# stormalex/minimap2_chaindp

Hardware: AMD Instinct MI355X
Metric: chained anchors/sec (whole node) (higher is better)
Workload: dtype int32

## Files before the change

minimap2_chaindp_amd/csrc/chaindp_lanes.h:

```cpp
#ifndef CHAINDP_LANES_H
#define CHAINDP_LANES_H

#include <hip/hip_runtime.h>
#include <stdint.h>

namespace chaindp {

#if defined(__HIP_DEVICE_COMPILE__)
#define TW_LDS(T, a) ((__attribute__((address_space(3))) T*)(a))
#else
#define TW_LDS(T, a) ((T*)(uintptr_t)(a))
#endif
#if defined(__HIP_DEVICE_COMPILE__)
#define TW_CONST(T, p) ((const __attribute__((address_space(4))) T*)(uintptr_t)(p))
#else
#define TW_CONST(T, p) ((const T*)(p))
#endif
typedef uint32_t tw_u32x2 __attribute__((ext_vector_type(2)));
typedef uint32_t tw_u32x4 __attribute__((ext_vector_type(4)));

__device__ __forceinline__ tw_u32x2 tw_ld64(uint32_t a) { return *TW_LDS(const tw_u32x2, a); }
__device__ __forceinline__ int tw_ld32(uint32_t a) { return *TW_LDS(const int, a); }
__device__ __forceinline__ int tw_ld_i8(uint32_t a) { return (int)*TW_LDS(const signed char, a); }
__device__ __forceinline__ int tw_ld_u8(uint32_t a) { return (int)*TW_LDS(const unsigned char, a); }
__device__ __forceinline__ tw_u32x4 tw_ld128(uint32_t a) { return *TW_LDS(const tw_u32x4, a); }
__device__ __forceinline__ void tw_st64(uint32_t a, uint32_t x, uint32_t y) { tw_u32x2 t; t.x = x; t.y = y; *TW_LDS(tw_u32x2, a) = t; }
__device__ __forceinline__ void tw_st32(uint32_t a, int v) { *TW_LDS(int, a) = v; }
__device__ __forceinline__ void tw_st8(uint32_t a, int v) { *TW_LDS(signed char, a) = (signed char)v; }
__device__ __forceinline__ void tw_st128(uint32_t a, uint32_t x, uint32_t y, uint32_t z, uint32_t w) { tw_u32x4 t; t.x = x; t.y = y; t.z = z; t.w = w; *TW_LDS(tw_u32x4, a) = t; }

#if defined(__HIP_DEVICE_COMPILE__)
#define TW_VREG(x) asm volatile("" : "+v"(x))
#else
#define TW_VREG(x) ((void)(x))
#endif

#define TW_UNI(x) ((uint32_t)__builtin_amdgcn_readfirstlane((int)(x)))

__device__ __forceinline__ uint32_t tw_sad(uint32_t a, uint32_t b, uint32_t c)
{
	uint32_t d = 0;
#if defined(__HIP_DEVICE_COMPILE__)
	asm("v_sad_u32 %0, %1, %2, %3" : "=v"(d) : "v"(a), "v"(b), "v"(c));
#endif
	return d;
}

__device__ __forceinline__ uint32_t tw_absdiff(uint32_t a, uint32_t b)
{
	uint32_t d = 0;
#if defined(__HIP_DEVICE_COMPILE__)
	asm("v_sad_u32 %0, %1, %2, 0" : "=v"(d) : "v"(a), "v"(b));
#endif
	return d;
}

__device__ __forceinline__ uint32_t tw_sub_m1(uint32_t b, uint32_t a)
{
	uint32_t d = 0;
#if defined(__HIP_DEVICE_COMPILE__)
	asm("v_xad_u32 %0, %1, -1, %2" : "=v"(d) : "v"(a), "v"(b));
#endif
	return d;
}

#define TW_ULT(a, b) __builtin_amdgcn_uicmp((unsigned)(a), (unsigned)(b), 36)
#define TW_EQ(a, b)  __builtin_amdgcn_uicmp((unsigned)(a), (unsigned)(b), 32)
#define TW_SGT(a, b) __builtin_amdgcn_sicmp((int)(a), (int)(b), 38)
#define TW_SGE(a, b) __builtin_amdgcn_sicmp((int)(a), (int)(b), 39)
#define TW_SEL(m, a, b) (__builtin_amdgcn_inverse_ballot_w64(m) ? (a) : (b))

}
#endif
```

minimap2_chaindp_amd/csrc/chaindp_twin.hip:

```cpp
#include <hip/hip_runtime.h>
#include <stdint.h>
#include <limits.h>
#include <stdio.h>
#include <stdlib.h>
#include <vector>
#include "chaindp_kernels.h"
#include "chaindp_wave.h"
#include "chaindp_lanes.h"

namespace chaindp {

#define TW_XY 0u
#define TW_PF 2048u
#define TW_V 3072u
#define TW_LUT_BYTES 512u
#define TW_ST_HALF 56u
#define TW_MK_HALF 260u
template <bool ONE_LUT> struct TwLayout {
	static constexpr bool HAS_XQ = !ONE_LUT;
	static constexpr uint32_t XQ = 3584u, XQ_HALF = 512u;
	static constexpr uint32_t LUT = ONE_LUT ? 3584u : XQ + 2u * XQ_HALF;
	static constexpr uint32_t LUT_HALF = ONE_LUT ? 0u : TW_LUT_BYTES;
	static constexpr uint32_t ST = LUT + (ONE_LUT ? 1u : 2u) * TW_LUT_BYTES;
	static constexpr uint32_t MK = ST + 2u * TW_ST_HALF;
	static constexpr uint32_t SP = MK + 2u * TW_MK_HALF;
	static constexpr uint32_t SP_HALF = ONE_LUT ? 0u : 64u;
	static constexpr uint32_t SP_OF_XQ = SP - XQ / 8u;
	static constexpr uint32_t KEY = SP + 128u;
	static constexpr uint32_t KEY_HALF = ONE_LUT ? 0u : 4u;
	static constexpr uint32_t BYTES = KEY + 8u;
	static_assert(ST % 8u == 0u && MK % 4u == 0u && KEY % 4u == 0u, "cold state is read as 64-bit words, marks and keys as 32-bit");
};
static_assert(TwLayout<true>::BYTES == 4864u && TwLayout<true>::BYTES <= 5120u, "one table: 32 workgroups per CU");
static_assert(TwLayout<false>::BYTES == 6400u, "two tables: 24 workgroups per CU");
template <bool SAMEGAP, bool ONE_LUT> struct TwWaves { static constexpr int N = !ONE_LUT ? 6 : SAMEGAP ? 8 : 7; };
#define TW_TILE 64
#define TW_RING 64
#define TW_QCH 8

__device__ __forceinline__ int tw_excl_max32(int v)
{
	v = max(v, __builtin_amdgcn_update_dpp(0, v, DPP_ROW_SHR(1), 0xf, 0xf, true));
	v = max(v, __builtin_amdgcn_update_dpp(0, v, DPP_ROW_SHR(2), 0xf, 0xf, true));
	v = max(v, __builtin_amdgcn_update_dpp(0, v, DPP_ROW_SHR(4), 0xf, 0xf, true));
	v = max(v, __builtin_amdgcn_update_dpp(0, v, DPP_ROW_SHR(8), 0xf, 0xf, true));
	int e = __builtin_amdgcn_update_dpp(0, v, DPP_ROW_SHR(1), 0xf, 0xf, true);
#if defined(__HIP_DEVICE_COMPILE__)
	asm("s_nop 1\n\tv_max_i32_dpp %0, %1, %0 row_bcast:15 row_mask:0xa bank_mask:0xf" : "+v"(e) : "v"(v));
#endif
	return e;
}
__device__ __forceinline__ int tw_incl_min32(int v)
{
	v = min(v, dpp_or_old<DPP_ROW_SHR(1), 0xf>(INT_MAX, v));
	v = min(v, dpp_or_old<DPP_ROW_SHR(2), 0xf>(INT_MAX, v));
	v = min(v, dpp_or_old<DPP_ROW_SHR(4), 0xf>(INT_MAX, v));
	v = min(v, dpp_or_old<DPP_ROW_SHR(8), 0xf>(INT_MAX, v));
	v = min(v, dpp_or_old<DPP_ROW_BCAST15, 0xa>(INT_MAX, v));
	return v;
}

__device__ __forceinline__ int tw_below_in_half(uint64_t m, bool hi_half)
{
	const int lo = (int)__builtin_amdgcn_mbcnt_lo((uint32_t)m, 0u);
	const int hi = (int)__builtin_amdgcn_mbcnt_hi((uint32_t)(m >> 32), 0u);
	return hi_half ? hi : lo;
}

__device__ __forceinline__ uint64_t tw_smear_halves(uint64_t m)
{
	uint32_t lo = 0, hi = 0;
#if defined(__HIP_DEVICE_COMPILE__)
	asm("s_cmp_lg_u32 %2, 0\n\ts_cselect_b32 %0, -1, 0\n\ts_cmp_lg_u32 %3, 0\n\ts_cselect_b32 %1, -1, 0"
	    : "=&s"(lo), "=&s"(hi) : "s"(TW_UNI((uint32_t)m)), "s"(TW_UNI((uint32_t)(m >> 32))) : "scc");
#endif
	return (uint64_t)hi << 32 | lo;
}

__device__ __forceinline__ uint64_t tw_last_or_lane0(uint64_t m)
{
	uint32_t lo = 0, hi = 0;
#if defined(__HIP_DEVICE_COMPILE__)
	asm("s_flbit_i32_b32 %0, %2\n\ts_flbit_i32_b32 %1, %3\n\ts_lshr_b32 %0, 0x80000000, %0\n\ts_lshr_b32 %1, 0x80000000, %1"
	    : "=&s"(lo), "=&s"(hi) : "s"(TW_UNI((uint32_t)m)), "s"(TW_UNI((uint32_t)(m >> 32))));
#endif
	return (uint64_t)hi << 32 | lo;
}

__device__ __forceinline__ uint32_t tw_both_halves(uint64_t m)
{
	uint32_t t = 0;
#if defined(__HIP_DEVICE_COMPILE__)
	asm("s_cmp_lg_u32 %1, 0\n\ts_cselect_b32 %0, %2, 0" : "=s"(t) : "s"(TW_UNI((uint32_t)m)), "s"(TW_UNI((uint32_t)(m >> 32))) : "scc");
#endif
	return t;
}

__device__ __forceinline__ uint64_t tw_below_first(uint64_t m, uint64_t b)
{
	const uint32_t blo = (uint32_t)b, bhi = (uint32_t)(b >> 32);
	const uint32_t klo = blo ? (blo & (0u - blo)) - 1u : 0xffffffffu, khi = bhi ? (bhi & (0u - bhi)) - 1u : 0xffffffffu;
	return m & ((uint64_t)khi << 32 | klo);
}

#define TW_HI31 0x8000000080000000ull

struct TwinArgs {
	Params par;
	const int64_t *off;
	const ulonglong2 *a;
	const unsigned long long *sumq;
	const uint16_t *lut;
	int lut_stride;
	const Unit *units;
	const UnitAux *aux;
	const unsigned long long *counters;
	int32_t *f, *p, *v;
	int32_t *first_child;
	uint8_t *flags;
	Unit *left;
	unsigned int *left_cnt;
	unsigned int *queue;
	const unsigned int *key_range;
	unsigned int *route;
	int two_tables;
	int force_left;
	int64_t total;
	unsigned long long *stamp;
};

struct TwinCold {
	int64_t next;
	int64_t base;
	uint64_t x_carry;
	int32_t rel0, room, read, tile0;
};

struct TwinHot {
	uint32_t S;
	uint32_t m4;
	uint32_t pc;
	uint32_t pend;
};
#define TW_CARRY 40u

#ifdef CHAINDP_TWIN_STAMPS
#define TW_STAMP(...) __VA_ARGS__
#else
#define TW_STAMP(...)
#endif
#if defined(CHAINDP_TWIN_STAMPS) && CHAINDP_TWIN_STAMPS == 2
#define TW_STAMP_A(...)
#define TW_STAMP_B(...) __VA_ARGS__
#elif defined(CHAINDP_TWIN_STAMPS) && CHAINDP_TWIN_STAMPS == 1
#define TW_STAMP_A(...) __VA_ARGS__
#define TW_STAMP_B(...)
#else
#define TW_STAMP_A(...)
#define TW_STAMP_B(...)
#endif
#if defined(CHAINDP_TWIN_STAMPS) && CHAINDP_TWIN_STAMPS == 3
#define TW_STAMP_C(...) __VA_ARGS__
#else
#define TW_STAMP_C(...)
#endif
#define TW_NOW() __builtin_amdgcn_s_memtime()

template <bool SAMEGAP, bool ONE_LUT>
__global__ __launch_bounds__(64) __attribute__((amdgpu_waves_per_eu(TwWaves<SAMEGAP, ONE_LUT>::N, TwWaves<SAMEGAP, ONE_LUT>::N))) void k_chain_twin(TwinArgs g)
{
	using L = TwLayout<ONE_LUT>;
	const int lane = threadIdx.x;
	const bool hi_half = lane >= 32;
	const int h = lane >> 5, hl = lane & 31;

	uint32_t L16 = (uint32_t)hl << 4;
	const uint32_t mkbase = L::MK + TW_MK_HALF * (uint32_t)h;
	const uint32_t curbase = L::XQ + L::XQ_HALF * (uint32_t)h;
	uint32_t c_mkbase = mkbase;
	uint32_t c_far = mkbase + 256u;
	uint32_t c_own = mkbase + ((uint32_t)hl << 2);
	uint32_t c_lut = ONE_LUT ? 0u : L::LUT + L::LUT_HALF * (uint32_t)h;
	uint32_t c_8h = (uint32_t)h << 3;
	uint32_t c_M = (uint32_t)g.par.max_dist_x;
	uint32_t c_bw = (uint32_t)g.par.bw;
	uint32_t c_cbw = c_M - 1u > c_bw ? c_M - 1u - c_bw : 0u;
	const uint32_t mdq = (uint32_t)(g.par.max_dist_x < g.par.max_dist_y ? g.par.max_dist_x : g.par.max_dist_y);
	uint32_t c_dqoff = c_M - mdq;
	int c_ms = g.par.max_skip;
	int c_min = INT_MIN;
	int c_Mout = hl == 31 ? g.par.max_dist_x : INT_MAX;
	uint32_t c_bwl = c_bw + c_lut;
	uint32_t c_cbwl = c_cbw - c_lut;
	constexpr uint32_t LUT_OFF = ONE_LUT ? L::LUT : 0u;
	TW_VREG(L16); TW_VREG(c_far); TW_VREG(c_own);
	if (!ONE_LUT) { TW_VREG(c_M); TW_VREG(c_ms); }
	if (!ONE_LUT) TW_VREG(c_lut);
	if (!SAMEGAP) TW_VREG(c_dqoff);
	TW_VREG(c_min); TW_VREG(c_Mout); TW_VREG(c_bwl); TW_VREG(c_cbwl);

	const uint64_t maxx = (uint64_t)(int64_t)g.par.max_dist_x;
	const uint32_t route = *g.route;
	if (ONE_LUT ? route == 1u || g.key_range[0] != g.key_range[1] || g.two_tables : route == 1u || route == 2u) return;
	const int64_t n_units = (int64_t)(uint32_t)g.counters[0];
	const int64_t n_single = (int64_t)(g.counters[0] >> 32);
	const bool short_units = (g.total - n_single) <= 512 * n_units;
	if (!short_units) {
		if (blockIdx.x == 0 && lane == 0) *g.left_cnt = 0xffffffffu;
		return;
	}
	if (blockIdx.x == 0 && lane == 0) *g.route = ONE_LUT ? 2u : 3u;
	const bool params_ok = g.lut != nullptr && !g.par.is_cdna && g.par.max_dist_x >= 1 && g.par.max_dist_y >= 0 &&
	                       ((uint64_t)(int64_t)g.par.max_dist_x + 1) * 129ull < (1ull << 31) && g.par.bw + 1 <= (int)TW_LUT_BYTES && g.force_left != 1;

	TwinHot u;
	u.S = 0; u.m4 = 0; u.pc = L::HAS_XQ ? curbase : 0u; u.pend = u.pc;
	uint64_t live_m = ~0ull;
	uint64_t contm = 0;
	const uint32_t st_addr = L::ST + TW_ST_HALF * (uint32_t)h;
#define TW_COLD (*TW_LDS(TwinCold, st_addr))
	const uint32_t xcd = blockIdx.x & 7u;
	const uint32_t n_halves = 2u * gridDim.x;
#ifndef TW_END_UNITS
#define TW_END_UNITS 16u
#define TW_PIECE 1u
#endif
	const uint32_t U1 = n_units > (long long)TW_END_UNITS * n_halves ? ((uint32_t)n_units - TW_END_UNITS * n_halves) & ~(8u * TW_QCH - 1u) : 0u;
	const uint32_t G1k = U1 / (8u * TW_QCH);
	auto grab = [&](uint32_t p, uint32_t &nx, uint32_t &ne) {
		if (p < G1k) { nx = (8u * p + xcd) * TW_QCH; ne = nx + TW_QCH; }
		else { nx = U1 + TW_PIECE * (8u * (p - G1k) + xcd); ne = nx + TW_PIECE; }
	};
	if (hl == 0) {
		uint32_t nx, ne;
		grab(((blockIdx.x >> 3) << 1) | (uint32_t)h, nx, ne);
		tw_st64(st_addr, nx, ne); tw_st64(st_addr + 8u, 0u, 0u);
		tw_st64(st_addr + 16u, 0u, 0u); tw_st64(st_addr + 24u, 0u, 0u);
		tw_st64(st_addr + 32u, 0u, (uint32_t)-TW_TILE);
		tw_st64(st_addr + TW_CARRY, 0xfffffffcu, 0u); tw_st64(st_addr + TW_CARRY + 8u, 0u, 0u);
		tw_st32(L::KEY + 4u * (uint32_t)h, -1);
	}
	wave_mem_fence();

	constexpr bool PF = !ONE_LUT;
	uint64_t nx0_x = 0, nx0_y = 0, nx1_x = 0, nx1_y = 0;
	int32_t pfu0 = -1, pfu1 = -1;

	TW_STAMP(unsigned long long st_t0 = 0; unsigned int st_service = 0, st_n_service = 0, st_n_fast = 0, st_flush = 0, st_unit = 0, st_n_unit = 0, st_head = 0, st_take = 0, st_tail = 0;)

	auto service = [&](uint64_t svc) {
#if defined(__HIP_DEVICE_COMPILE__)
		asm volatile("s_waitcnt vmcnt(0)" ::: "memory");
#endif
		wave_mem_fence();
		uint64_t retired = 0;
		for (int hs = 0; hs < 2; ++hs) {
			if (((svc >> (32 * hs)) & 1ull) == 0) continue;
			TW_STAMP_B(const unsigned long long th0 = g.stamp ? TW_NOW() : 0;)
			const uint64_t hm = hs ? 0xffffffff00000000ull : 0x00000000ffffffffull;
			const uint32_t sa = L::ST + TW_ST_HALF * (uint32_t)hs, keya = L::KEY + L::KEY_HALF * (uint32_t)hs;
			const uint32_t mkb = L::MK + TW_MK_HALF * (uint32_t)hs, lutb = L::LUT + L::LUT_HALF * (uint32_t)hs;
			const uint32_t curb = L::XQ + L::XQ_HALF * (uint32_t)hs, spb = L::SP + L::SP_HALF * (uint32_t)hs;
			const tw_u32x2 cw0 = tw_ld64(sa), cw1 = tw_ld64(sa + 8u), cw2 = tw_ld64(sa + 16u), cw3 = tw_ld64(sa + 24u), cw4 = tw_ld64(sa + 32u);
			int64_t c_next = (int64_t)((uint64_t)TW_UNI(cw0.y) << 32 | TW_UNI(cw0.x));
			int64_t c_base = (int64_t)((uint64_t)TW_UNI(cw1.y) << 32 | TW_UNI(cw1.x));
			uint64_t c_xcarry = (uint64_t)TW_UNI(cw2.y) << 32 | TW_UNI(cw2.x);
			int c_rel0 = (int)TW_UNI(cw3.x), c_room = (int)TW_UNI(cw3.y), c_read = (int)TW_UNI(cw4.x), c_tile0 = (int)TW_UNI(cw4.y);
			auto tile_cnt = [&]() -> int {
				const uint32_t pe = TW_UNI(__builtin_amdgcn_readlane((int)u.pend, 32 * hs));
				if constexpr (L::HAS_XQ) return (int)((pe - curb) >> 3);
				else return pe < mkb ? 0 : (int)((pe - mkb) >> 2) + 1 - c_tile0;
			};
			const int cnt_prev = tile_cnt();
			const int slow_h = (int)TW_UNI((uint32_t)tw_ld32(sa + TW_CARRY + 12u));
			const uint32_t cur_key = TW_UNI((uint32_t)tw_ld32(keya));
			const int tile_prev = c_tile0, rel0_prev = c_rel0;
			const int64_t base_prev = c_base;
			bool live = true;
			const uint32_t nx0 = (uint32_t)c_next, ne0 = (uint32_t)((uint64_t)c_next >> 32);
			tw_u32x4 rec0 = {0u, 0u, 0u, 0u}, aux0 = {0u, 0u, 0u, 0u}, rec1 = {0u, 0u, 0u, 0u};
			const bool rec0_ok = nx0 < ne0 && (int64_t)nx0 < n_units;
			const bool rec1_ok = PF && rec0_ok && nx0 + 1u < ne0 && (int64_t)nx0 + 1 < n_units;
			if (rec0_ok) { rec0 = *TW_CONST(tw_u32x4, g.units + nx0); aux0 = *TW_CONST(tw_u32x4, g.aux + nx0); }
			if (rec1_ok) rec1 = *TW_CONST(tw_u32x4, g.units + nx0 + 1u);

			auto take_tile = [&](const uint64_t an_x, const uint64_t an_y) -> int {
				const int i_lane = c_tile0 + lane;
				const bool have = i_lane < c_room;
				uint64_t xp;
				{
					uint32_t lo = (uint32_t)wave_shift_up1((int)(uint32_t)an_x, 0), hi = (uint32_t)wave_shift_up1((int)(uint32_t)(an_x >> 32), 0);
					if (lane == 0) { lo = (uint32_t)c_xcarry; hi = (uint32_t)(c_xcarry >> 32); }
					xp = (uint64_t)hi << 32 | lo;
				}
				const bool stop = !have || (i_lane > 0 && an_x - xp > maxx);
				const uint64_t stop_m = __builtin_amdgcn_ballot_w64(stop);
				const int cnt = stop_m ? __builtin_ctzll(stop_m) : TW_TILE;
				c_xcarry = readlane_u64(an_x, 63);
				if constexpr (L::HAS_XQ) { u.pc = TW_SEL(hm, curb, u.pc); u.pend = TW_SEL(hm, curb + ((uint32_t)cnt << 3), u.pend); }
				else u.pend = TW_SEL(hm, mkb + ((uint32_t)(c_tile0 + cnt - 1) << 2), u.pend);
				if (cnt == 0) return 0;
				wave_mem_fence();
				if (lane < cnt) {
					const int sp = span_of_hi((uint32_t)(an_y >> 32));
					tw_st64((((uint32_t)i_lane & 127u) << 4 | (uint32_t)hs << 3) + TW_XY, (uint32_t)an_x + 1u, (uint32_t)an_y + 1u);
					if constexpr (L::HAS_XQ) {
						tw_st64(curb + ((uint32_t)lane << 3), (uint32_t)an_x, (uint32_t)an_y);
						tw_st8(spb + (uint32_t)lane, sp - 1);
					} else tw_st8((((uint32_t)i_lane & 63u) << 1 | (uint32_t)hs) + L::SP, sp - 1);
					g.first_child[c_base + i_lane] = NO_CHILD;
				}
				wave_mem_fence();
				if constexpr (PF) {
					if (cnt == TW_TILE && c_tile0 + TW_TILE < c_room) {
						uint64_t rx = 0, ry = 0;
						if (i_lane + TW_TILE < c_room) { const ulonglong2 t = g.a[c_base + i_lane + TW_TILE]; rx = t.x; ry = t.y; }
						if (hs) { nx1_x = rx; nx1_y = ry; pfu1 = -1; } else { nx0_x = rx; nx0_y = ry; pfu0 = -1; }
					}
				}
				return cnt;
			};

			bool goes_on = cnt_prev == TW_TILE && c_tile0 + TW_TILE < c_room;
			if (goes_on && (slow_h * 8 > c_tile0 + TW_TILE || g.force_left == 2)) {
				if (lane == 0) {
					Unit un; un.start = (int64_t)((uint64_t)c_base | (uint64_t)(uint32_t)(c_tile0 + TW_TILE) << 32); un.read = c_read; un.len = c_room;
					g.left[atomicAdd(g.left_cnt, 1u)] = un;
				}
				goes_on = false;
			}
			if (goes_on) {
				c_tile0 += TW_TILE;
				uint64_t nt_x = 0, nt_y = 0;
				if constexpr (PF) { nt_x = hs ? nx1_x : nx0_x; nt_y = hs ? nx1_y : nx0_y; }
				else if (c_tile0 + lane < c_room) { const ulonglong2 t = g.a[c_base + c_tile0 + lane]; nt_x = t.x; nt_y = t.y; }
				if (take_tile(nt_x, nt_y) == 0) goes_on = false;
			}
			TW_STAMP_B(if (g.stamp) st_take += (unsigned int)(TW_NOW() - th0);)
			TW_STAMP_A(const unsigned long long tf0 = g.stamp ? TW_NOW() : 0;)
			if (cnt_prev > 0) {
				const int i_lane = tile_prev + lane;
				const bool have = lane < cnt_prev;
				const int64_t gi = base_prev + i_lane;
				int fi = 0, p4 = -4;
				if (have) {
					const tw_u32x2 pf = tw_ld64((((uint32_t)i_lane & 63u) << 4 | (uint32_t)hs << 3) + TW_PF);
					p4 = (int)pf.x; fi = (int)pf.y + 1;
				}
				const int pi = p4 >> 2;
				int val = fi, ptr = have ? pi : -1;
				const bool ext = ptr >= 0 && ptr < tile_prev;
				int vext = 0;
				if (ext) {
					vext = tw_ld32((((uint32_t)ptr & 63u) << 3 | (uint32_t)hs << 2) + TW_V);
					val = max(val, vext & 0x7fffffff);
					ptr = -1;
				}
				const bool ext_self = ext && vext < 0;
				for (int r = 0; r < 6; ++r) {
					if (__builtin_amdgcn_ballot_w64(ptr >= tile_prev) == 0) break;
					const int src = (ptr >= tile_prev ? ptr - tile_prev : lane) << 2;
					const int pv = __builtin_amdgcn_ds_bpermute(src, val);
					const int pp = __builtin_amdgcn_ds_bpermute(src, ptr);
					if (ptr >= tile_prev) { val = max(val, pv); ptr = pp; }
				}
				const bool self = val >= g.par.min_sc || pi >= 0;
				const int srcp = (pi >= tile_prev ? pi - tile_prev : lane) << 2;
				const int pself_in = __builtin_amdgcn_ds_bpermute(srcp, self ? 1 : 0);
				const bool pred_self = ext ? ext_self : pself_in != 0;
				wave_mem_fence();
				if (have) tw_st32((((uint32_t)i_lane & 63u) << 3 | (uint32_t)hs << 2) + TW_V, val | (self ? INT_MIN : 0));
				wave_mem_fence();
				if (have) {
					g.f[gi] = fi;
					g.p[gi] = pi < 0 ? -1 : pi + rel0_prev;
					g.v[gi] = val;
					int maybe_first = 0;
					if (pi >= 0 && !pred_self) { atomicMin(&g.first_child[base_prev + pi], rel0_prev + i_lane); maybe_first = 4; }
					g.flags[gi] = (uint8_t)((self ? 2 : 0) | maybe_first | (val >= g.par.min_sc ? 8 : 0) | (fi < val ? 16 : 0));
				}
			}
			TW_STAMP_A(if (g.stamp) st_flush += (unsigned int)(TW_NOW() - tf0);)
			TW_STAMP_A(const unsigned long long tu0 = g.stamp ? TW_NOW() : 0;)
			TW_STAMP_A(if (g.stamp && !goes_on) ++st_n_unit;)
			bool have_rec = rec0_ok;
			const bool rec0_used = !goes_on;
			uint32_t cur_key_now = cur_key;
			while (!goes_on && live) {
				uint32_t nx = (uint32_t)c_next, ne = (uint32_t)((uint64_t)c_next >> 32);
				if (nx >= ne) {
					uint32_t q0 = 0;
					if (lane == 0) q0 = atomicAdd(g.queue + 64u * xcd, 1u);
					grab(TW_UNI(q0), nx, ne);
					have_rec = false;
				}
				if ((int64_t)nx >= n_units) {
					c_next = (int64_t)((uint64_t)ne << 32 | nx); live = false;
					if constexpr (L::HAS_XQ) { u.pc = TW_SEL(hm, curb, u.pc); u.pend = TW_SEL(hm, curb, u.pend); }
					else u.pend = TW_SEL(hm, 0u, u.pend);
					break;
				}
				TW_STAMP_C(const unsigned long long tc0 = g.stamp ? TW_NOW() : 0;)
				if (!have_rec) { rec0 = *TW_CONST(tw_u32x4, g.units + nx); aux0 = *TW_CONST(tw_u32x4, g.aux + nx); }
				have_rec = false;
				TW_STAMP_C(if (g.stamp) { asm volatile("" :: "s"(rec0.x), "s"(aux0.x)); st_head += (unsigned int)(TW_NOW() - tc0); })
				c_next = (int64_t)((uint64_t)ne << 32 | (nx + 1u));
				Unit un;
				un.start = (int64_t)((uint64_t)rec0.y << 32 | rec0.x); un.read = (int32_t)rec0.z; un.len = (int32_t)rec0.w;
				if (!params_ok || (aux0.z & 1u) || g.par.n_segs > 1 || (ONE_LUT && cur_key_now != 0xffffffffu && aux0.y != cur_key_now)) {
					if (lane == 0) g.left[atomicAdd(g.left_cnt, 1u)] = un;
					continue;
				}
				c_base = un.start; c_rel0 = (int)aux0.x; c_room = un.len; c_read = un.read; c_tile0 = 0;
				uint64_t tl_x = 0, tl_y = 0;
				TW_STAMP_C(const unsigned long long tc1 = g.stamp ? TW_NOW() : 0;)
				TW_STAMP_C(if (g.stamp && PF && (hs ? pfu1 : pfu0) == (int32_t)c_base) ++st_n_unit;)
				if (PF && (hs ? pfu1 : pfu0) == (int32_t)c_base) { tl_x = hs ? nx1_x : nx0_x; tl_y = hs ? nx1_y : nx0_y; }
				else if (lane < c_room) { const ulonglong2 t = g.a[c_base + lane]; tl_x = t.x; tl_y = t.y; }
				if constexpr (PF) { if (hs) pfu1 = -1; else pfu0 = -1; }
				TW_STAMP_C(if (g.stamp) { asm volatile("" :: "v"(tl_x), "v"(tl_y)); asm volatile("s_waitcnt vmcnt(0)" ::: "memory"); st_take += (unsigned int)(TW_NOW() - tc1); })
				TW_STAMP_C(const unsigned long long tc2 = g.stamp ? TW_NOW() : 0;)
				wave_mem_fence();
				if (aux0.y != cur_key_now) {
					const uint2 *src = (const uint2*)(g.lut + (int64_t)c_read * g.lut_stride);
					for (int k = lane; k * 4 <= g.par.bw; k += 64) {
						const uint2 t = src[k];
						const uint32_t w = (t.x & 0xffu) | (t.x >> 8 & 0xff00u) | (t.y << 16 & 0xff0000u) | (t.y << 8 & 0xff000000u);
						tw_st32(lutb + ((uint32_t)k << 2), (int)w);
					}
					cur_key_now = aux0.y;
					if (lane == 0) tw_st32(keya, (int)cur_key_now);
				}
				const uint32_t x_none = (uint32_t)__builtin_amdgcn_readlane((int)(uint32_t)tl_x, 0) - (uint32_t)maxx - 1u;
				for (int k = lane; k < 128; k += 64) tw_st64(((uint32_t)k << 4 | (uint32_t)hs << 3) + TW_XY, x_none, 0u);
				for (int k = lane; k < 65; k += 64) tw_st32(mkb + ((uint32_t)k << 2), -1);
				wave_mem_fence();
				c_xcarry = 0;
				if (lane == 0) tw_st32(sa + TW_CARRY + 12u, 0);
				if (take_tile(tl_x, tl_y) > 0) goes_on = true;
				TW_STAMP_C(if (g.stamp) { st_tail += (unsigned int)(TW_NOW() - tc2); ++st_unit; })
			}
			if (PF && live) {
				const int cnt_now = tile_cnt();
				const uint32_t nxn = (uint32_t)c_next, nen = (uint32_t)((uint64_t)c_next >> 32);
				if (!(cnt_now == TW_TILE && c_tile0 + TW_TILE < c_room) && (hs ? pfu1 : pfu0) < 0 && nxn < nen && (int64_t)nxn < n_units &&
				    ((nxn == nx0 && rec0_ok && !rec0_used) || (nxn == nx0 + 1u && rec1_ok))) {
					const tw_u32x4 rn = nxn == nx0 ? rec0 : rec1;
					const int32_t st = (int32_t)rn.x, ln = (int32_t)rn.w;
					uint64_t rx = 0, ry = 0;
					if (lane < ln) { const ulonglong2 t = g.a[(int64_t)st + lane]; rx = t.x; ry = t.y; }
					if (hs) { nx1_x = rx; nx1_y = ry; pfu1 = st; } else { nx0_x = rx; nx0_y = ry; pfu0 = st; }
				}
			}
			TW_STAMP_A(if (g.stamp) st_unit += (unsigned int)(TW_NOW() - tu0);)
			if (live) {
				const uint32_t i = (uint32_t)c_tile0;
				u.S = TW_SEL(hm, (i - 1u) << 4 | (uint32_t)hs << 3, u.S); u.m4 = TW_SEL(hm, ((i - 1u) << 2) + mkb, u.m4);
			} else retired |= hm;
			if (lane == 0) {
				tw_st64(sa, (uint32_t)c_next, (uint32_t)((uint64_t)c_next >> 32)); tw_st64(sa + 8u, (uint32_t)c_base, (uint32_t)((uint64_t)c_base >> 32));
				tw_st64(sa + 16u, (uint32_t)c_xcarry, (uint32_t)(c_xcarry >> 32)); tw_st64(sa + 24u, (uint32_t)c_rel0, (uint32_t)c_room);
				tw_st64(sa + 32u, (uint32_t)c_read, (uint32_t)c_tile0);
			}
		}
		wave_mem_fence();
		live_m &= ~retired;
		contm &= ~svc;
	};

	auto slow_tail = [&](uint64_t D, uint32_t a_cur, int nskip_after) -> uint64_t {
		const uint64_t giveup = ~D & contm;
		const int vlast = __builtin_amdgcn_ds_bpermute(((h << 5) + 31) << 2, nskip_after);
		wave_mem_fence();
		const tw_u32x2 cur = tw_ld64(a_cur);
		if (__builtin_amdgcn_inverse_ballot_w64(D)) {
			u.m4 += 4u;
			u.S = ((u.m4 - c_mkbase) << 2) | c_8h;
			if constexpr (L::HAS_XQ) u.pc += 8u;
		} else {
			if (hl == 0) {
				tw_st64(st_addr + TW_CARRY, cur.x, cur.y);
				tw_st32(st_addr + TW_CARRY + 8u, vlast);
				tw_st32(st_addr + TW_CARRY + 12u, tw_ld32(st_addr + TW_CARRY + 12u) + 1);
			}
			u.S -= 512u;
		}
		contm = ~D & ~giveup & live_m;
		if (__builtin_expect(giveup != 0, 0)) {
			if (__builtin_amdgcn_inverse_ballot_w64(giveup)) {
				wave_mem_fence();
				if (hl == 0) {
					const TwinCold c = TW_COLD;
					Unit un; un.start = (int64_t)((uint64_t)c.base | (uint64_t)(uint32_t)c.tile0 << 32); un.read = c.read; un.len = c.room;
					g.left[atomicAdd(g.left_cnt, 1u)] = un;
				}
				u.pc = curbase; u.pend = L::HAS_XQ ? curbase : 0u;
			}
			return giveup;
		}
		return 0;
	};

	TW_STAMP(if (g.stamp) st_t0 = TW_NOW();)
	service(~0ull);
	bool force_general = false;
	while (live_m != 0) {
		wave_mem_fence();
		uint64_t svc = 0;
		if (__builtin_expect(contm == 0 && live_m == ~0ull && !force_general, 1)) {
			uint64_t B, X, tile;
			int cB;
			uint32_t a_cur;
			for (;;) {
				const uint32_t t0 = u.S - L16;
				const uint32_t S1 = u.S + 16u;
				const tw_u32x2 xy = tw_ld64((t0 & 0x7f8u) + TW_XY);
				const tw_u32x2 cur = tw_ld64(L::HAS_XQ ? u.pc : (S1 & 0x7f8u) + TW_XY);
#if defined(__HIP_DEVICE_COMPILE__)
				__builtin_amdgcn_sched_barrier(0);
#endif
				const tw_u32x2 pf = tw_ld64((t0 & 0x3f8u) + TW_PF);
				const int spm1 = tw_ld_u8(L::HAS_XQ ? (u.pc >> 3) + L::SP_OF_XQ : __builtin_amdgcn_ubfe(S1, 3, 7) + L::SP);
				const uint32_t drm1 = L::HAS_XQ ? cur.x - xy.x : tw_sub_m1(cur.x, xy.x), dqm1 = L::HAS_XQ ? cur.y - xy.y : tw_sub_m1(cur.y, xy.y);
				const uint32_t ddl = ONE_LUT ? tw_absdiff(drm1, dqm1) : tw_sad(drm1, dqm1, c_lut);
				const uint32_t dqs = SAMEGAP ? dqm1 : __builtin_elementwise_add_sat(dqm1, c_dqoff);
				const uint32_t m3 = max(max(drm1, dqs), ddl + c_cbwl);
				const uint64_t okm = TW_ULT(m3, c_M);
				const uint32_t dst = TW_SEL(okm, min(u.m4 - pf.x, c_far), c_far);
				tw_st32(dst, (int)u.m4);
				wave_mem_fence();
				const int tj = tw_ld32(c_own);
				const int lutv = tw_ld_i8(min(ddl, c_bwl) + LUT_OFF);
#if defined(__HIP_DEVICE_COMPILE__)
				__builtin_amdgcn_sched_barrier(0);
#endif
				const int sc0 = min(min((int)dqm1, (int)drm1), spm1);
				const int sc = TW_SEL(okm, sc0 + (int)pf.y + lutv, c_min);
				const int excl = max(tw_excl_max32(sc), spm1);
				const uint64_t A = TW_SGT(sc, excl);
				B = TW_EQ(tj, u.m4) & okm & ~A;
				const uint64_t OUT = TW_SGE(drm1, c_Mout);
				cB = tw_below_in_half(B, hi_half);
				tile = 0; X = 0; a_cur = 0;
				if (__builtin_expect((TW_SGT(cB, 0) & A) != 0, 0)) { force_general = true; break; }
				a_cur = S1 & 0x3f8u;
				{
					const uint32_t wp = TW_SEL(A, u.m4 - c_own, 0xfffffffcu);
					const int wf = TW_SEL(A, sc, spm1);
					if (__builtin_amdgcn_inverse_ballot_w64(tw_last_or_lane0(A))) tw_st64(a_cur + TW_PF, wp, (uint32_t)wf);
				}
				X = (TW_SGE(cB, c_ms) & B) | OUT;
				if (__builtin_expect(tw_both_halves(X) == 0, 0)) break;
				u.m4 += 4u; u.S = S1;
				if constexpr (L::HAS_XQ) { u.pc += 8u; tile = TW_SGE(u.pc, u.pend); }
				else tile = TW_SGE(u.m4, u.pend);
				TW_STAMP(if (g.stamp) ++st_n_fast;)
				if (__builtin_expect(tile != 0, 0)) break;
				wave_mem_fence();
			}
			if (!force_general && tile == 0) {
				svc = slow_tail(tw_smear_halves(X), a_cur + TW_PF, cB + (int)__builtin_amdgcn_inverse_ballot_w64(B));
			}
		} else {
			force_general = false;
			const uint32_t t0 = u.S - L16;
			const uint32_t xcur = ((((u.m4 - c_mkbase) + 4u) << 2) & 0x7f8u) | c_8h;
			const tw_u32x2 xy = tw_ld64((t0 & 0x7f8u) + TW_XY);
			const tw_u32x2 pf = tw_ld64((t0 & 0x3f8u) + TW_PF);
			const tw_u32x2 cur = tw_ld64(L::HAS_XQ ? u.pc : xcur + TW_XY);
			const int spm1 = tw_ld_u8(L::HAS_XQ ? (u.pc >> 3) + L::SP_OF_XQ : ((xcur >> 3) & 0x7fu) + L::SP);
			const uint64_t first = ~contm;
			const tw_u32x2 carry = tw_ld64(st_addr + TW_CARRY);
			const int maxf = TW_SEL(first, spm1, (int)carry.y);
			const uint32_t maxj4 = TW_SEL(first, 0xfffffffcu, carry.x);
			const int nskip0 = TW_SEL(first, 0, tw_ld32(st_addr + TW_CARRY + 8u));
			const uint32_t kb4 = TW_SEL(first, 0u, 128u);
			const uint32_t drm1 = L::HAS_XQ ? cur.x - xy.x : tw_sub_m1(cur.x, xy.x), dqm1 = L::HAS_XQ ? cur.y - xy.y : tw_sub_m1(cur.y, xy.y);
			const uint32_t ddl = ONE_LUT ? tw_absdiff(drm1, dqm1) : tw_sad(drm1, dqm1, c_lut);
			const uint32_t dqs = SAMEGAP ? dqm1 : __builtin_elementwise_add_sat(dqm1, c_dqoff);
			const uint32_t m3 = max(max(drm1, dqs), ddl + c_cbwl);
			const uint64_t okm = TW_ULT(m3, c_M) & ~(contm & TW_HI31) & live_m;
			const int sc0 = min(min((int)dqm1, (int)drm1), spm1);
			const int lutv = tw_ld_i8(min(ddl, c_bwl) + LUT_OFF);
			const uint32_t dst = TW_SEL(okm, min(u.m4 - pf.x, c_far), c_far);
			tw_st32(dst, (int)u.m4);
			wave_mem_fence();
			const int tj = tw_ld32(c_own + kb4);
			const int sc = TW_SEL(okm, sc0 + (int)pf.y + lutv, c_min);
			const int excl = max(tw_excl_max32(sc), maxf);
			const uint64_t A = TW_SGT(sc, excl);
			const uint64_t B = TW_EQ(tj, u.m4) & okm & ~A;
			const uint64_t OUT = TW_SGE(drm1, c_M);
			const int cB = tw_below_in_half(B, hi_half), cA = tw_below_in_half(A, hi_half);
			const int isA = (int)__builtin_amdgcn_inverse_ballot_w64(A), isB = (int)__builtin_amdgcn_inverse_ballot_w64(B);
			const uint64_t inter = TW_SGT(cB, 0) & A;
			uint64_t brk, Ap;
			int nskip_after;
			if (inter == 0) {
				nskip_after = max(nskip0 - cA - isA, 0) + cB + isB;
				brk = TW_SGT(nskip_after, c_ms) & B;
				Ap = A;
			} else {
				const int Sk = nskip0 + cB + isB - cA - isA;
				nskip_after = Sk - min(tw_incl_min32(Sk), 0);
				brk = TW_SGT(nskip_after, c_ms) & B;
				Ap = tw_below_first(A, brk);
			}
			const uint32_t a_cur = (xcur & 0x3f8u) + TW_PF;
			{
				const uint32_t wp = TW_SEL(Ap, u.m4 - c_own - kb4, maxj4);
				const int wf = TW_SEL(Ap, sc, maxf);
				if (__builtin_amdgcn_inverse_ballot_w64(tw_last_or_lane0(Ap))) tw_st64(a_cur, wp, (uint32_t)wf);
			}
			const uint64_t D = tw_smear_halves(brk | (OUT & TW_HI31) | ~live_m);
			svc = slow_tail(D, a_cur, nskip_after);
		}
		svc |= tw_smear_halves((L::HAS_XQ ? TW_SGE(u.pc, u.pend) : TW_SGE(u.m4, u.pend)) & live_m & ~contm);
		if (__builtin_expect(svc != 0, 0)) {
			TW_STAMP(const unsigned long long ts = g.stamp ? TW_NOW() : 0;)
			service(svc & live_m);
			TW_STAMP(if (g.stamp) { st_service += (unsigned int)(TW_NOW() - ts); ++st_n_service; })
		}
	}
	TW_STAMP(if (g.stamp && lane == 0) {
		unsigned long long *o = g.stamp + 12 * (size_t)blockIdx.x;
		o[0] = TW_NOW() - st_t0; o[1] = st_service; o[2] = st_flush; o[3] = st_unit; o[4] = st_n_service; o[5] = st_n_fast; o[6] = st_n_unit; o[7] = 1; o[8] = st_head; o[9] = st_take; o[10] = st_tail;
	})
#undef TW_COLD
}

size_t twin_lds_bytes(bool one_table) { return one_table ? TwLayout<true>::BYTES : TwLayout<false>::BYTES; }

int twin_max_wg_per_cu(bool samegap, bool one_table)
{
	const int lds_wg = one_table ? 32 : 24;
	const int waves = one_table ? (samegap ? TwWaves<true, true>::N : TwWaves<false, true>::N)
	                            : (samegap ? TwWaves<true, false>::N : TwWaves<false, false>::N);
	return 4 * waves < lds_wg ? 4 * waves : lds_wg;
}

template <bool ONE_LUT>
static hipError_t launch_twin_layout(hipStream_t st, TwinArgs g, int64_t max_units, int cus, unsigned int *d_queue)
{
	const bool samegap = g.par.max_dist_y >= g.par.max_dist_x;
	const int max_wg = twin_max_wg_per_cu(samegap, ONE_LUT);
	int64_t blocks = (max_units + 2 * TW_QCH - 1) / (2 * TW_QCH);
	static const int wg_env = getenv("CHAINDP_TWIN_WG_PER_CU") ? atoi(getenv("CHAINDP_TWIN_WG_PER_CU")) : 0;
	const int64_t cap = (int64_t)cus * (wg_env >= 1 && wg_env <= max_wg ? wg_env : max_wg);
	if (blocks > cap) blocks = cap;
	if (blocks < 1) blocks = 1;
	blocks = (blocks + 7) & ~(int64_t)7;
	{
		const hipError_t e = hipMemsetD32Async((hipDeviceptr_t)d_queue, (int)(2 * blocks / 8), 8 * 64, st);
		if (e != hipSuccess) return e;
	}
	static unsigned long long *d_stamp = nullptr;
	const bool stamp = getenv("CHAINDP_TWIN_STAMP") != nullptr;
	if (stamp && !d_stamp && hipMalloc((void**)&d_stamp, (size_t)cap * 96) != hipSuccess) d_stamp = nullptr;
	g.stamp = stamp ? d_stamp : nullptr;
	if (g.stamp) (void)hipMemsetAsync(d_stamp, 0, (size_t)blocks * 96, st);
	{
		hipFuncAttributes fa;
		const void *fn = samegap ? (const void*)k_chain_twin<true, ONE_LUT> : (const void*)k_chain_twin<false, ONE_LUT>;
		const hipError_t e = hipFuncGetAttributes(&fa, fn);
		if (e != hipSuccess) return e;
		if (fa.sharedSizeBytes != 0) return hipErrorInvalidConfiguration;
	}
	if (samegap) hipLaunchKernelGGL((k_chain_twin<true, ONE_LUT>), dim3((unsigned)blocks), dim3(64), TwLayout<ONE_LUT>::BYTES, st, g);
	else hipLaunchKernelGGL((k_chain_twin<false, ONE_LUT>), dim3((unsigned)blocks), dim3(64), TwLayout<ONE_LUT>::BYTES, st, g);
	if (g.stamp) {
		std::vector<unsigned long long> hb((size_t)blocks * 12);
		if (hipStreamSynchronize(st) == hipSuccess && hipMemcpy(hb.data(), d_stamp, hb.size() * 8, hipMemcpyDeviceToHost) == hipSuccess) {
			double tot = 0, svc = 0, flush = 0, unit = 0, nsvc = 0, nfast = 0, nunit = 0, nb = 0, head = 0, take = 0, tail = 0;
			for (int64_t b = 0; b < blocks; ++b) if (hb[(size_t)b * 12 + 7]) {
				const unsigned long long *o = &hb[(size_t)b * 12];
				tot += o[0]; svc += o[1]; flush += o[2]; unit += o[3]; nsvc += o[4]; nfast += o[5]; nunit += o[6]; head += o[8]; take += o[9]; tail += o[10]; ++nb;
			}
			if (nb > 0) fprintf(stderr, "[twin stamp raw] sums over waves: head %.0f take %.0f tail %.0f unit %.0f n_unit %.0f (build 3: ticks until the record / the first tile / the rest of a unit switch; switches; first tiles requested ahead)\n", head, take, tail, unit, nunit);
			if (nb > 0) fprintf(stderr, "[twin stamp] %.0f waves, %.0f ticks each: service %.1f%% (%.0f calls, %.0f ticks each: cold state and decisions %.0f, next tile %.0f, flush %.0f, "
			                "unit switch %.0f (%.0f switches, %.0f ticks each), first anchor and cold state back %.0f), passes %.0f (%.0f ticks each, everything else included)\n",
			        nb, tot / nb, 100.0 * svc / tot, nsvc, svc / (nsvc > 0 ? nsvc : 1), head / (nsvc > 0 ? nsvc : 1), take / (nsvc > 0 ? nsvc : 1), flush / (nsvc > 0 ? nsvc : 1),
			        unit / (nsvc > 0 ? nsvc : 1), nunit, unit / (nunit > 0 ? nunit : 1), tail / (nsvc > 0 ? nsvc : 1), nfast, (tot - svc) / (nfast > 0 ? nfast : 1));
		}
	}
	return hipGetLastError();
}

hipError_t launch_chain_twin(hipStream_t st, const Params &par, int64_t max_units, const int64_t *d_off, const void *d_a,
                             const unsigned long long *d_sumq, const uint16_t *d_lut, int lut_stride, const Unit *d_units,
                             const unsigned long long *d_counters, int32_t *d_f, int32_t *d_p, int32_t *d_v,
                             int32_t *d_first_child, uint8_t *d_flags, Unit *d_left, unsigned int *d_left_cnt, int force_left, int64_t total,
                             const UnitAux *d_unit_aux, const unsigned int *d_key_range, unsigned int *d_route, unsigned int *d_queue, int two_tables)
{
	if (max_units <= 0) return hipSuccess;
	if (!d_unit_aux || !d_key_range || !d_route || !d_queue) return hipErrorInvalidValue;
	int dev = 0, cus = 256;
	if (hipGetDevice(&dev) == hipSuccess) (void)hipDeviceGetAttribute(&cus, hipDeviceAttributeMultiprocessorCount, dev);
	TwinArgs g;
	g.par = par; g.off = d_off; g.a = (const ulonglong2*)d_a; g.sumq = d_sumq; g.lut = d_lut; g.lut_stride = lut_stride;
	g.units = d_units; g.aux = d_unit_aux; g.counters = d_counters; g.f = d_f; g.p = d_p; g.v = d_v; g.first_child = d_first_child; g.flags = d_flags;
	g.left = d_left; g.left_cnt = d_left_cnt; g.queue = d_queue; g.key_range = d_key_range; g.route = d_route; g.two_tables = two_tables != 0;
	g.force_left = force_left; g.total = total; g.stamp = nullptr;
	hipError_t e = launch_twin_layout<true>(st, g, max_units, cus, d_queue);
	if (e == hipSuccess) e = launch_twin_layout<false>(st, g, max_units, cus, d_queue);
	return e;
}

}
```

Measured before the change: 21.29 billion.

## Restructure ONE_LUT fast loop with precomputed pass count and exec-masked PF store

For the ONE_LUT variant, the fast anchor loop now computes up front how many passes remain before the tile ends, using readlane on both halves, instead of comparing per iteration. The conflict test becomes a scalar negate-and-mask (tw_above_first), and the skip-count check uses popcount of B per half, so the full exit mask is built only when a half may hit max_skip. The PF write is done with inline asm that saves exec, writes, then restores it, replacing a branch on a lane predicate. L16 and S are rebased by one step so each iteration uses S1 directly. The aim is fewer vector ops and branches per step on the serial DP chain, at the cost of hand-written asm and more complex index bookkeeping.

```diff
diff --git a/minimap2_chaindp_amd/csrc/chaindp_lanes.h b/minimap2_chaindp_amd/csrc/chaindp_lanes.h
--- a/minimap2_chaindp_amd/csrc/chaindp_lanes.h
+++ b/minimap2_chaindp_amd/csrc/chaindp_lanes.h
@@ -33,6 +33,12 @@
 #define TW_VREG(x) asm volatile("" : "+v"(x))
 #else
 #define TW_VREG(x) ((void)(x))
+#endif
+
+#if defined(__HIP_DEVICE_COMPILE__)
+#define TW_OPAQUE(x) asm("" : "+v"(x))
+#else
+#define TW_OPAQUE(x) ((void)(x))
 #endif
 
 #define TW_UNI(x) ((uint32_t)__builtin_amdgcn_readfirstlane((int)(x)))
diff --git a/minimap2_chaindp_amd/csrc/chaindp_twin.hip b/minimap2_chaindp_amd/csrc/chaindp_twin.hip
--- a/minimap2_chaindp_amd/csrc/chaindp_twin.hip
+++ b/minimap2_chaindp_amd/csrc/chaindp_twin.hip
@@ -105,6 +105,27 @@
 
 #define TW_HI31 0x8000000080000000ull
 
+__device__ __forceinline__ uint64_t tw_above_first(uint64_t a, uint64_t b)
+{
+	uint32_t lo = 0, hi = 0;
+#if defined(__HIP_DEVICE_COMPILE__)
+	asm("s_sub_i32 %0, 0, %2\n\ts_sub_i32 %1, 0, %3" : "=&s"(lo), "=&s"(hi) : "s"(TW_UNI((uint32_t)b)), "s"(TW_UNI((uint32_t)(b >> 32))) : "scc");
+#endif
+	return a & ((uint64_t)hi << 32 | lo);
+}
+
+__device__ __forceinline__ void tw_st64_pf_lanes(uint64_t m, uint32_t a, uint32_t x, uint32_t y)
+{
+#if defined(__HIP_DEVICE_COMPILE__)
+	tw_u32x2 t; t.x = x; t.y = y;
+	uint64_t saved;
+	asm volatile("s_and_saveexec_b64 %0, %1\n\tds_write_b64 %2, %3 offset:2048\n\ts_mov_b64 exec, %0"
+	             : "=&s"(saved) : "s"(m), "v"(a), "v"(t) : "memory", "scc");
+#endif
+}
+static_assert(TW_PF == 2048u, "tw_st64_pf_lanes writes the PF ring at DS offset 2048");
+
+
 struct TwinArgs {
 	Params par;
 	const int64_t *off;
@@ -174,7 +195,7 @@
 	const bool hi_half = lane >= 32;
 	const int h = lane >> 5, hl = lane & 31;
 
-	uint32_t L16 = (uint32_t)hl << 4;
+	uint32_t L16 = ((uint32_t)hl + 1u) << 4;
 	const uint32_t mkbase = L::MK + TW_MK_HALF * (uint32_t)h;
 	const uint32_t curbase = L::XQ + L::XQ_HALF * (uint32_t)h;
 	uint32_t c_mkbase = mkbase;
@@ -508,62 +529,135 @@
 		wave_mem_fence();
 		uint64_t svc = 0;
 		if (__builtin_expect(contm == 0 && live_m == ~0ull && !force_general, 1)) {
-			uint64_t B, X, tile;
-			int cB;
-			uint32_t a_cur;
-			for (;;) {
-				const uint32_t t0 = u.S - L16;
-				const uint32_t S1 = u.S + 16u;
-				const tw_u32x2 xy = tw_ld64((t0 & 0x7f8u) + TW_XY);
-				const tw_u32x2 cur = tw_ld64(L::HAS_XQ ? u.pc : (S1 & 0x7f8u) + TW_XY);
-#if defined(__HIP_DEVICE_COMPILE__)
-				__builtin_amdgcn_sched_barrier(0);
-#endif
-				const tw_u32x2 pf = tw_ld64((t0 & 0x3f8u) + TW_PF);
-				const int spm1 = tw_ld_u8(L::HAS_XQ ? (u.pc >> 3) + L::SP_OF_XQ : __builtin_amdgcn_ubfe(S1, 3, 7) + L::SP);
-				const uint32_t drm1 = L::HAS_XQ ? cur.x - xy.x : tw_sub_m1(cur.x, xy.x), dqm1 = L::HAS_XQ ? cur.y - xy.y : tw_sub_m1(cur.y, xy.y);
-				const uint32_t ddl = ONE_LUT ? tw_absdiff(drm1, dqm1) : tw_sad(drm1, dqm1, c_lut);
-				const uint32_t dqs = SAMEGAP ? dqm1 : __builtin_elementwise_add_sat(dqm1, c_dqoff);
-				const uint32_t m3 = max(max(drm1, dqs), ddl + c_cbwl);
-				const uint64_t okm = TW_ULT(m3, c_M);
-				const uint32_t dst = TW_SEL(okm, min(u.m4 - pf.x, c_far), c_far);
-				tw_st32(dst, (int)u.m4);
-				wave_mem_fence();
-				const int tj = tw_ld32(c_own);
-				const int lutv = tw_ld_i8(min(ddl, c_bwl) + LUT_OFF);
-#if defined(__HIP_DEVICE_COMPILE__)
-				__builtin_amdgcn_sched_barrier(0);
-#endif
-				const int sc0 = min(min((int)dqm1, (int)drm1), spm1);
-				const int sc = TW_SEL(okm, sc0 + (int)pf.y + lutv, c_min);
-				const int excl = max(tw_excl_max32(sc), spm1);
-				const uint64_t A = TW_SGT(sc, excl);
-				B = TW_EQ(tj, u.m4) & okm & ~A;
-				const uint64_t OUT = TW_SGE(drm1, c_Mout);
-				cB = tw_below_in_half(B, hi_half);
-				tile = 0; X = 0; a_cur = 0;
-				if (__builtin_expect((TW_SGT(cB, 0) & A) != 0, 0)) { force_general = true; break; }
-				a_cur = S1 & 0x3f8u;
-				{
-					const uint32_t wp = TW_SEL(A, u.m4 - c_own, 0xfffffffcu);
-					const int wf = TW_SEL(A, sc, spm1);
-					if (__builtin_amdgcn_inverse_ballot_w64(tw_last_or_lane0(A))) tw_st64(a_cur + TW_PF, wp, (uint32_t)wf);
-				}
-				X = (TW_SGE(cB, c_ms) & B) | OUT;
-				if (__builtin_expect(tw_both_halves(X) == 0, 0)) break;
-				u.m4 += 4u; u.S = S1;
-				if constexpr (L::HAS_XQ) { u.pc += 8u; tile = TW_SGE(u.pc, u.pend); }
-				else tile = TW_SGE(u.m4, u.pend);
-				TW_STAMP(if (g.stamp) ++st_n_fast;)
-				if (__builtin_expect(tile != 0, 0)) break;
-				wave_mem_fence();
-			}
-			if (!force_general && tile == 0) {
-				svc = slow_tail(tw_smear_halves(X), a_cur + TW_PF, cB + (int)__builtin_amdgcn_inverse_ballot_w64(B));
+			if constexpr (ONE_LUT) {
+				uint64_t B, D = 0;
+				bool tile_end = false;
+				int npass = 1;
+				if constexpr (L::HAS_XQ) {
+					const int n0 = (int)(TW_UNI(__builtin_amdgcn_readlane((int)u.pend, 0)) - TW_UNI(__builtin_amdgcn_readlane((int)u.pc, 0))) >> 3;
+					const int n1 = (int)(TW_UNI(__builtin_amdgcn_readlane((int)u.pend, 32)) - TW_UNI(__builtin_amdgcn_readlane((int)u.pc, 32))) >> 3;
+					npass = max(min(n0, n1), 1);
+				} else {
+					const int n0 = (int)(TW_UNI(__builtin_amdgcn_readlane((int)u.pend, 0)) - TW_UNI(__builtin_amdgcn_readlane((int)u.m4, 0))) >> 2;
+					const int n1 = (int)(TW_UNI(__builtin_amdgcn_readlane((int)u.pend, 32)) - TW_UNI(__builtin_amdgcn_readlane((int)u.m4, 32))) >> 2;
+					npass = max(min(n0, n1), 1);
+				}
+				const uint32_t ms0 = (uint32_t)max(g.par.max_skip, 0);
+				u.S += 16u;
+				for (;;) {
+					const uint32_t S1 = u.S;
+					const uint32_t t0 = S1 - L16;
+					const tw_u32x2 xy = tw_ld64((t0 & 0x7f8u) + TW_XY);
+					const tw_u32x2 cur = tw_ld64(L::HAS_XQ ? u.pc : (S1 & 0x7f8u) + TW_XY);
+	#if defined(__HIP_DEVICE_COMPILE__)
+					__builtin_amdgcn_sched_barrier(0);
+	#endif
+					const tw_u32x2 pf = tw_ld64((t0 & 0x3f8u) + TW_PF);
+					uint32_t a_cur = S1 & 0x3f8u;
+					TW_OPAQUE(a_cur);
+					const int spm1 = tw_ld_u8(L::HAS_XQ ? (u.pc >> 3) + L::SP_OF_XQ : (a_cur >> 3) + L::SP);
+	#ifdef TW_EXP_PAD
+					for (int k = 0; k < TW_EXP_PAD; ++k) { uint32_t pad; asm volatile("v_max3_u32 %0, %1, %1, %1" : "=v"(pad) : "v"(c_far)); }
+	#endif
+					const uint32_t drm1 = L::HAS_XQ ? cur.x - xy.x : tw_sub_m1(cur.x, xy.x), dqm1 = L::HAS_XQ ? cur.y - xy.y : tw_sub_m1(cur.y, xy.y);
+					const uint32_t ddl = ONE_LUT ? tw_absdiff(drm1, dqm1) : tw_sad(drm1, dqm1, c_lut);
+					const uint32_t dqs = SAMEGAP ? dqm1 : __builtin_elementwise_add_sat(dqm1, c_dqoff);
+					const uint32_t m3 = max(max(drm1, dqs), ddl + c_cbwl);
+					const uint64_t okm = TW_ULT(m3, c_M);
+					const uint32_t dst = TW_SEL(okm, min(u.m4 - pf.x, c_far), c_far);
+					tw_st32(dst, (int)u.m4);
+					wave_mem_fence();
+					const int tj = tw_ld32(c_own);
+					const int lutv = tw_ld_i8(min(ddl, c_bwl) + LUT_OFF);
+	#if defined(__HIP_DEVICE_COMPILE__)
+					__builtin_amdgcn_sched_barrier(0);
+	#endif
+					const int sc0 = min(min((int)dqm1, (int)drm1), spm1);
+					const int sc = TW_SEL(okm, sc0 + (int)pf.y + lutv, c_min);
+					const int excl = max(tw_excl_max32(sc), spm1);
+					const uint64_t A = TW_SGT(sc, excl);
+					B = TW_EQ(tj, u.m4) & okm & ~A;
+					const uint32_t blo = (uint32_t)B, bhi = (uint32_t)(B >> 32);
+					if (__builtin_expect(tw_above_first(A, B) != 0, 0)) { force_general = true; break; }
+					{
+						const uint32_t wp = TW_SEL(A, u.m4 - c_own, 0xfffffffcu);
+						const int wf = max(excl, sc);
+						tw_st64_pf_lanes(tw_last_or_lane0(A), a_cur, wp, (uint32_t)wf);
+					}
+					const uint32_t nlo = (uint32_t)__builtin_popcount(blo), nhi = (uint32_t)__builtin_popcount(bhi);
+					if (__builtin_expect(min(nlo, nhi) <= ms0, 0)) {
+						const uint64_t OUT = TW_SGE(drm1, c_Mout);
+						D = tw_smear_halves(OUT | (nlo > ms0 ? 0x00000000ffffffffull : 0ull) | (nhi > ms0 ? 0xffffffff00000000ull : 0ull));
+						if (__builtin_expect(tw_both_halves(D) == 0, 0)) break;
+					}
+					u.m4 += 4u; u.S += 16u;
+					if constexpr (L::HAS_XQ) u.pc += 8u;
+					TW_STAMP(if (g.stamp) ++st_n_fast;)
+					if (__builtin_expect(--npass <= 0, 0)) { tile_end = true; break; }
+					wave_mem_fence();
+				}
+				const uint32_t a_cur = u.S & 0x3f8u;
+				u.S -= 16u;
+				if (!force_general && !tile_end) {
+					svc = slow_tail(D, a_cur + TW_PF, tw_below_in_half(B, hi_half) + (int)__builtin_amdgcn_inverse_ballot_w64(B));
+				}
+			} else {
+				uint64_t B, X, tile;
+				int cB;
+				uint32_t a_cur;
+				for (;;) {
+					const uint32_t S1 = u.S + 16u;
+					const uint32_t t0 = S1 - L16;
+					const tw_u32x2 xy = tw_ld64((t0 & 0x7f8u) + TW_XY);
+					const tw_u32x2 cur = tw_ld64(u.pc);
+	#if defined(__HIP_DEVICE_COMPILE__)
+					__builtin_amdgcn_sched_barrier(0);
+	#endif
+					const tw_u32x2 pf = tw_ld64((t0 & 0x3f8u) + TW_PF);
+					const int spm1 = tw_ld_u8((u.pc >> 3) + L::SP_OF_XQ);
+					const uint32_t drm1 = cur.x - xy.x, dqm1 = cur.y - xy.y;
+					const uint32_t ddl = tw_sad(drm1, dqm1, c_lut);
+					const uint32_t dqs = SAMEGAP ? dqm1 : __builtin_elementwise_add_sat(dqm1, c_dqoff);
+					const uint32_t m3 = max(max(drm1, dqs), ddl + c_cbwl);
+					const uint64_t okm = TW_ULT(m3, c_M);
+					const uint32_t dst = TW_SEL(okm, min(u.m4 - pf.x, c_far), c_far);
+					tw_st32(dst, (int)u.m4);
+					wave_mem_fence();
+					const int tj = tw_ld32(c_own);
+					const int lutv = tw_ld_i8(min(ddl, c_bwl) + LUT_OFF);
+	#if defined(__HIP_DEVICE_COMPILE__)
+					__builtin_amdgcn_sched_barrier(0);
+	#endif
+					const int sc0 = min(min((int)dqm1, (int)drm1), spm1);
+					const int sc = TW_SEL(okm, sc0 + (int)pf.y + lutv, c_min);
+					const int excl = max(tw_excl_max32(sc), spm1);
+					const uint64_t A = TW_SGT(sc, excl);
+					B = TW_EQ(tj, u.m4) & okm & ~A;
+					const uint64_t OUT = TW_SGE(drm1, c_Mout);
+					cB = tw_below_in_half(B, hi_half);
+					tile = 0; X = 0; a_cur = 0;
+					if (__builtin_expect((TW_SGT(cB, 0) & A) != 0, 0)) { force_general = true; break; }
+					a_cur = S1 & 0x3f8u;
+					{
+						const uint32_t wp = TW_SEL(A, u.m4 - c_own, 0xfffffffcu);
+						const int wf = TW_SEL(A, sc, spm1);
+						if (__builtin_amdgcn_inverse_ballot_w64(tw_last_or_lane0(A))) tw_st64(a_cur + TW_PF, wp, (uint32_t)wf);
+					}
+					X = (TW_SGE(cB, c_ms) & B) | OUT;
+					if (__builtin_expect(tw_both_halves(X) == 0, 0)) break;
+					u.m4 += 4u; u.S = S1;
+					u.pc += 8u; tile = TW_SGE(u.pc, u.pend);
+					TW_STAMP(if (g.stamp) ++st_n_fast;)
+					if (__builtin_expect(tile != 0, 0)) break;
+					wave_mem_fence();
+				}
+				if (!force_general && tile == 0) {
+					svc = slow_tail(tw_smear_halves(X), a_cur + TW_PF, cB + (int)__builtin_amdgcn_inverse_ballot_w64(B));
+				}
 			}
 		} else {
 			force_general = false;
-			const uint32_t t0 = u.S - L16;
+			const uint32_t t0 = u.S + 16u - L16;
 			const uint32_t xcur = ((((u.m4 - c_mkbase) + 4u) << 2) & 0x7f8u) | c_8h;
 			const tw_u32x2 xy = tw_ld64((t0 & 0x7f8u) + TW_XY);
 			const tw_u32x2 pf = tw_ld64((t0 & 0x3f8u) + TW_PF);
```

After: 21.81 billion (median of 6 runs). 1.02x the previous value.
